# nadeemlab/DeepLIIF

Measured on AMD Instinct MI355X. Metric: 512x512 tiles/s train-step (5G+5D), higher is better.
Workload: dtype bf16; 1 GPU; DeepLIIF train step, 5x Resnet-9block G + 5x NLayerD(n=4), GAN+SmoothL1+Adam (BASELINE configs[2] per GPU); tile=512x512x3, batch_per_gpu=8, global_batch=8, norm=instance, precision_policy=bf16, parallelism=dp1, rccl_ranks=1, backend=nccl, streams=3

## Files before the change

### deepliif_amd/csrc/conv_s2d.hip

```cpp
#include "conv_args.h"

typedef __attribute__((ext_vector_type(16))) float f32x16_t;
typedef __attribute__((address_space(3))) char lds_char_t;
typedef __attribute__((address_space(3))) const bf16x8_t lds_frag_t;

__device__ __attribute__((aligned(64))) unsigned char g_s2d_zero_page[64];

template <int V> struct S2DIC { static constexpr int value = V; };

struct S2dArgs {
    ConvArgs a;
    int R, nstrips, segs;
};

constexpr int S2D_EVEN = 128 * 128;
constexpr int S2D_ODD = 136 * 128;
constexpr int S2D_SLOT = S2D_EVEN + S2D_ODD;
constexpr int S2D_TILE = 4 * S2D_SLOT;
constexpr int S2D_BIAS = S2D_TILE + 64 * 256;
constexpr size_t S2D_LDS = (size_t)S2D_BIAS + 512;
static_assert(S2D_LDS <= 160 * 1024, "LDS of one CU");

__device__ __forceinline__ float s2d_row16_sum(float v) {
    v += __builtin_bit_cast(float, __builtin_amdgcn_update_dpp(0, __builtin_bit_cast(int, v), 0xB1, 0xf, 0xf, false));
    v += __builtin_bit_cast(float, __builtin_amdgcn_update_dpp(0, __builtin_bit_cast(int, v), 0x4E, 0xf, 0xf, false));
    v += __builtin_bit_cast(float, __builtin_amdgcn_update_dpp(0, __builtin_bit_cast(int, v), 0x141, 0xf, 0xf, false));
    v += __builtin_bit_cast(float, __builtin_amdgcn_update_dpp(0, __builtin_bit_cast(int, v), 0x140, 0xf, 0xf, false));
    return v;
}

template <bool STATS, bool RELU>
__global__ void __launch_bounds__(256) conv_s2d_kernel(const S2dArgs sa) {
    const ConvArgs &a = sa.a;
    extern __shared__ __attribute__((aligned(16))) char smem_raw[];
    lds_char_t *lds = (lds_char_t *)smem_raw;

    const int tid = threadIdx.x, lane = tid & 63;
    const int wave = __builtin_amdgcn_readfirstlane(tid >> 6);
    const int lr = lane & 31, lh = lane >> 5;

    int b = blockIdx.x;
    const int strip = b % sa.nstrips; b /= sa.nstrips;
    const int seg = b % sa.segs; b /= sa.segs;
    const int tn = b % a.tiles_n;
    const int n = b / a.tiles_n;
    const int ho0 = strip * sa.R;

    bf16x8_t W[3][3][4];
    {
        const bf16_t *wp = a.w_hi + (size_t)(tn * 128 + wave * 32 + lr) * a.w_kstride + a.phase_kbase[0] + lh * 8;
#pragma unroll
        for (int kh = 0; kh < 3; ++kh)
#pragma unroll
            for (int kw = 0; kw < 3; ++kw)
#pragma unroll
                for (int s = 0; s < 4; ++s) W[kh][kw][s] = *reinterpret_cast<const bf16x8_t *>(wp + (kh * 3 + kw) * 64 + s * 16);
    }

    const int lrow = lane >> 3, lcp = lane & 7;
    const char *in = reinterpret_cast<const char *>(a.in);
    const int psb = a.in_pstride * 2;
    const unsigned OOB = 0x80000000u;
    const int pp0 = 8 * wave + lrow;
    const unsigned swz = (unsigned)((lcp ^ ((pp0 >> 1) & 7)) * 16);
    const unsigned o_off = (unsigned)((seg * 256 + 2 * pp0) * psb) + swz;
    const unsigned e_off = o_off + (unsigned)psb;
    const unsigned o_off0 = (seg * 256 + 2 * pp0 - 1 >= 0) ? o_off : OOB;
    const unsigned o_off4 = (lrow == 0) ? o_off : OOB;
    const size_t row_bytes = (size_t)a.Wi * psb;
    const __amdgpu_buffer_rsrc_t rsrc_in = __builtin_amdgcn_make_buffer_rsrc(const_cast<char *>(in + (size_t)n * a.Hi * row_bytes - psb), 0, 0x7fffffff, 0x00020000);

    const __amdgpu_buffer_rsrc_t rsrc_none = __builtin_amdgcn_make_buffer_rsrc(const_cast<char *>(in), 0, 0, 0x00020000);
    auto stage_piece = [&](auto Kc, int soff, int slot, const __amdgpu_buffer_rsrc_t rsrc_in) __attribute__((always_inline)) {
        constexpr int K = decltype(Kc)::value;
        const int dst = slot * S2D_SLOT;
        if constexpr (K < 4) {
            __builtin_amdgcn_raw_ptr_buffer_load_lds(rsrc_in, (__attribute__((address_space(3))) void *)(lds + dst + (wave + 4 * K) * 1024), 16, (int)e_off,
                                                     soff + K * 64 * psb, 0, 0);
        } else if constexpr (K < 8) {
            __builtin_amdgcn_raw_ptr_buffer_load_lds(rsrc_in, (__attribute__((address_space(3))) void *)(lds + dst + S2D_EVEN + (wave + 4 * (K - 4)) * 1024), 16,
                                                     (int)(K == 4 ? o_off0 : o_off), soff + (K - 4) * 64 * psb, 0, 0);
        } else {
            if (wave == 0)
                __builtin_amdgcn_raw_ptr_buffer_load_lds(rsrc_in, (__attribute__((address_space(3))) void *)(lds + dst + S2D_EVEN + 16 * 1024), 16, (int)o_off4,
                                                         soff + 4 * 64 * psb, 0, 0);
        }
    };
    auto stage = [&](int r, int slot) __attribute__((always_inline)) {
        const int rowp = r * (int)row_bytes;
        stage_piece(S2DIC<0>{}, rowp, slot, rsrc_in); stage_piece(S2DIC<1>{}, rowp, slot, rsrc_in); stage_piece(S2DIC<2>{}, rowp, slot, rsrc_in);
        stage_piece(S2DIC<3>{}, rowp, slot, rsrc_in); stage_piece(S2DIC<4>{}, rowp, slot, rsrc_in); stage_piece(S2DIC<5>{}, rowp, slot, rsrc_in);
        stage_piece(S2DIC<6>{}, rowp, slot, rsrc_in); stage_piece(S2DIC<7>{}, rowp, slot, rsrc_in); stage_piece(S2DIC<8>{}, rowp, slot, rsrc_in);
    };

    const int a_kw1 = lr * 128 + ((lh ^ ((lr >> 1) & 7)) << 4);
    const int a_kw0 = S2D_EVEN + a_kw1;
    const int a_kw2 = S2D_EVEN + (lr + 1) * 128 + ((lh ^ (((lr + 1) >> 1) & 7)) << 4);

    f32x16_t accA[4], accB[4];

    auto frag_base = [&](int g_kw) __attribute__((always_inline)) { return g_kw == 0 ? a_kw0 : (g_kw == 1 ? a_kw1 : a_kw2); };
    auto read_group = [&](bf16x8_t (&F)[4], int addr) __attribute__((always_inline)) {
#pragma unroll
        for (int j = 0; j < 4; ++j) F[j] = *reinterpret_cast<lds_frag_t *>(lds + addr + j * 4096);
    };
    auto row_mac = [&](auto KHC, auto KHN, int slot, int slot_next, f32x16_t (&cur)[4], f32x16_t (&nxt)[4], bf16x8_t (&F0)[4], bf16x8_t (&F1)[4],
                       int soff_dma, int slot_dma, const __amdgpu_buffer_rsrc_t rsrc_dma) __attribute__((always_inline)) {
        constexpr int khc = decltype(KHC)::value, khn = decltype(KHN)::value;
        const int base = slot * S2D_SLOT;
        auto group = [&](auto Gc, bf16x8_t (&Fc)[4], bf16x8_t (&Fn)[4]) __attribute__((always_inline)) {
            constexpr int g = decltype(Gc)::value, kw = g >> 2, sx = g & 3;
            if constexpr (g + 1 < 12) read_group(Fn, base + (frag_base((g + 1) >> 2) ^ (((g + 1) & 3) << 5)));
            else if (slot_next >= 0) read_group(Fn, slot_next * S2D_SLOT + a_kw0);
            if constexpr (g < 9) stage_piece(S2DIC<(g < 9 ? g : 0)>{}, soff_dma, slot_dma, rsrc_dma);
#pragma unroll
            for (int j = 0; j < 4; ++j) {
                if constexpr (khc >= 0) cur[j] = dl_mfma32(W[khc < 0 ? 0 : khc][kw][sx], Fc[j], cur[j]);
                if constexpr (khn >= 0) nxt[j] = dl_mfma32(W[khn < 0 ? 0 : khn][kw][sx], Fc[j], nxt[j]);
            }
        };
        group(S2DIC<0>{}, F0, F1); group(S2DIC<1>{}, F1, F0); group(S2DIC<2>{}, F0, F1); group(S2DIC<3>{}, F1, F0);
        group(S2DIC<4>{}, F0, F1); group(S2DIC<5>{}, F1, F0); group(S2DIC<6>{}, F0, F1); group(S2DIC<7>{}, F1, F0);
        group(S2DIC<8>{}, F0, F1); group(S2DIC<9>{}, F1, F0); group(S2DIC<10>{}, F0, F1); group(S2DIC<11>{}, F1, F0);
    };

    float s1[8], s2[8];
#pragma unroll
    for (int e = 0; e < 8; ++e) { s1[e] = 0.f; s2[e] = 0.f; }
    lds_char_t *tile = lds + S2D_TILE;
    const int opb = a.out_pstride * 2;
    const __amdgpu_buffer_rsrc_t rsrc_out = __builtin_amdgcn_make_buffer_rsrc(reinterpret_cast<char *>(a.out) + (size_t)n * a.Ho * a.Wo * opb, 0, 0x7fffffff, 0x00020000);
    const unsigned st_off = (unsigned)((tid >> 4) * opb + (tn * 128 + (tid & 15) * 8) * 2);
    constexpr bool relu = RELU;
    __attribute__((address_space(3))) float *bias_l = reinterpret_cast<__attribute__((address_space(3))) float *>(lds + S2D_BIAS);
    if (tid < 128) {
        const int co = tn * 128 + tid;
        bias_l[tid] = (a.bias && co < a.bias_n) ? a.bias[co] : 0.f;
    }
    __syncthreads();
    auto reset_acc = [&](f32x16_t (&acc)[4]) __attribute__((always_inline)) {
        f32x4_t bv[4];
#pragma unroll
        for (int q = 0; q < 4; ++q) bv[q] = *reinterpret_cast<__attribute__((address_space(3))) const f32x4_t *>(bias_l + wave * 32 + q * 8 + lh * 4);
#pragma unroll
        for (int j = 0; j < 4; ++j)
#pragma unroll
            for (int r = 0; r < 16; ++r) acc[j][r] = bv[r >> 2][r & 3];
    };
    reset_acc(accA);
    reset_acc(accB);

    auto epilogue = [&](f32x16_t (&acc)[4], int ho) __attribute__((always_inline)) {
        const int orow = (ho * a.Wo + seg * 128) * opb;
#pragma unroll
        for (int h = 0; h < 2; ++h) {
#pragma unroll
            for (int jj = 0; jj < 2; ++jj) {
                const int j = 2 * h + jj;
#pragma unroll
                for (int q = 0; q < 4; ++q) {
                    float v[4];
#pragma unroll
                    for (int e = 0; e < 4; ++e) {
                        v[e] = acc[j][q * 4 + e];
                        if constexpr (relu) v[e] = v[e] > 0.f ? v[e] : 0.f;
                    }
                    u32x2_t pk;
                    pk[0] = pack2_bf16(v[0], v[1]);
                    pk[1] = pack2_bf16(v[2], v[3]);
                    const int unit = (wave * 8 + q * 2 + lh) ^ ((lr & 15) << 1);
                    *reinterpret_cast<__attribute__((address_space(3))) u32x2_t *>(tile + (jj * 32 + lr) * 256 + unit * 8) = pk;
                }
            }
            asm volatile("s_waitcnt lgkmcnt(0)\n\ts_barrier" ::: "memory");
#pragma unroll
            for (int it = 0; it < 4; ++it) {
                const int idx = tid + it * 256;
                const int row = idx >> 4, cc = idx & 15;
                const int unit = (cc * 2) ^ ((row & 15) << 1);
                const u32x4_t v = *reinterpret_cast<__attribute__((address_space(3))) const u32x4_t *>(tile + row * 256 + unit * 8);
                __builtin_amdgcn_raw_buffer_store_b128(v, rsrc_out, (int)st_off, orow + (h * 64 + it * 16) * opb, 0);
                if constexpr (STATS) {
#pragma unroll
                    for (int e = 0; e < 4; ++e) {
                        const float lo = h16_lo_f32(v[e]), hi = h16_hi_f32(v[e]);
                        s1[2 * e] += lo; s2[2 * e] += lo * lo; s1[2 * e + 1] += hi; s2[2 * e + 1] += hi * hi;
                    }
                }
            }
            asm volatile("s_waitcnt lgkmcnt(0)\n\ts_barrier" ::: "memory");
        }
        reset_acc(acc);
    };

    const int R = sa.R;
    const int r_first = 2 * ho0 - 1;
    bf16x8_t FA[4], FB[4];
    if (r_first >= 0) stage(r_first, 3);
    stage(2 * ho0, 0);
    stage(2 * ho0 + 1, 1);
    asm volatile("s_waitcnt vmcnt(0)\n\ts_barrier" ::: "memory");
    if (r_first >= 0) {
        read_group(FA, 3 * S2D_SLOT + a_kw0);
        row_mac(S2DIC<0>{}, S2DIC<-1>{}, 3, -1, accA, accB, FA, FB, 0, 2, rsrc_none);
        asm volatile("s_waitcnt lgkmcnt(0)\n\ts_barrier" ::: "memory");
    }
    auto out_row = [&](int t, int s0, f32x16_t (&cur)[4], f32x16_t (&nxt)[4]) __attribute__((always_inline)) {
        const int ho = ho0 + t;
        const bool more = t + 1 < R;
        const int soff = (2 * ho + 2) * (int)row_bytes;
        read_group(FA, s0 * S2D_SLOT + a_kw0);
        const __amdgpu_buffer_rsrc_t rs = more ? rsrc_in : rsrc_none;
        row_mac(S2DIC<1>{}, S2DIC<-1>{}, s0, s0 + 1, cur, nxt, FA, FB, soff, s0 ^ 2, rs);
        row_mac(S2DIC<2>{}, S2DIC<0>{}, s0 + 1, -1, cur, nxt, FA, FB, soff + (int)row_bytes, (s0 ^ 2) + 1, rs);
        __builtin_amdgcn_sched_barrier(0);
        epilogue(cur, ho);
        __builtin_amdgcn_sched_barrier(0);
        asm volatile("s_waitcnt vmcnt(8) lgkmcnt(0)\n\ts_barrier" ::: "memory");
    };
    for (int t = 0; t < R; t += 2) {
        out_row(t, 0, accA, accB);
        out_row(t + 1, 2, accB, accA);
    }

    if constexpr (STATS) {
        __attribute__((address_space(3))) float *red = reinterpret_cast<__attribute__((address_space(3))) float *>(tile);
#pragma unroll
        for (int e = 0; e < 8; ++e) {
            float t1 = s1[e], t2 = s2[e];
            t1 += __shfl_xor(t1, 16, 64); t2 += __shfl_xor(t2, 16, 64);
            t1 += __shfl_xor(t1, 32, 64); t2 += __shfl_xor(t2, 32, 64);
            if (lane < 16) { red[(wave * 2 + 0) * 128 + lane * 8 + e] = t1; red[(wave * 2 + 1) * 128 + lane * 8 + e] = t2; }
        }
        __syncthreads();
        if (tid < 128 && tn * 128 + tid < a.Co) {
            float t1 = 0.f, t2 = 0.f;
#pragma unroll
            for (int w = 0; w < 4; ++w) { t1 += red[(w * 2 + 0) * 128 + tid]; t2 += red[(w * 2 + 1) * 128 + tid]; }
            float *o = a.stats_part + ((size_t)(n * a.stats_nchunks + seg * sa.nstrips + strip) * 2) * a.Co + tn * 128 + tid;
            o[0] = t1;
            o[a.Co] = t2;
        }
    }
}

static int s2d_strip_rows(const ConvArgs &a) {
    const int segs = a.Wo / 128, tiles_n = a.Co / 128;
    const int per_img = a.N * segs * tiles_n;
    int best = 0;
    for (int R = 2; R <= a.Ho; R += 2) {
        if (a.Ho % R) continue;
        const int wgs = per_img * (a.Ho / R);
        if (best == 0 || wgs >= 240) best = R;
        if (wgs < 240) break;
    }
    return best;
}

bool s2d_eligible(const ConvArgs &a) {
    if (a.n_phase != 1 || a.splitk != 1 || a.raw_out || a.in_step != 2 || a.out_step != 1) return false;
    if (a.phase_tap_begin[1] - a.phase_tap_begin[0] != 9 || a.Ci != 64 || a.Co < 128 || (a.Co & 127)) return false;
    if (a.Hi != 2 * a.Ho || a.Wi != 2 * a.Wo || a.Hq != a.Ho || a.Wq != a.Wo || (a.Wo & 127) || (a.Ho & 1)) return false;
    if (a.pad_mode != DL_PAD_ZERO || a.bn_y != nullptr || a.in_act != DL_ACT_NONE || a.epi_old) return false;
    if (a.act != DL_ACT_NONE && a.act != DL_ACT_RELU) return false;
    for (int t = 0; t < 9; ++t) {
        const int dh = (int)(int8_t)(a.taps[t] & 0xff), dw = (int)(int8_t)((a.taps[t] >> 8) & 0xff);
        if (dh != t / 3 - 1 || dw != t % 3 - 1) return false;
    }
    return s2d_strip_rows(a) > 0;
}

int s2d_stats_chunks(const ConvArgs &a) {
    const int R = s2d_strip_rows(a);
    return R > 0 ? (a.Wo / 128) * (a.Ho / R) : 0;
}

int launch_conv_s2d(const ConvArgs &a0, hipStream_t stream) {
    S2dArgs sa;
    memset(&sa, 0, sizeof(sa));
    sa.a = a0;
    ConvArgs &a = sa.a;
    sa.R = s2d_strip_rows(a);
    if (sa.R <= 0) DL_FAIL("dl_conv_forward(s2d): no strip height for Ho=%d", a.Ho);
    sa.nstrips = a.Ho / sa.R;
    sa.segs = a.Wo / 128;
    a.tiles_n = a.Co / 128;
    a.tiles_m = a.N * sa.segs * sa.nstrips;
    if (a.stats_part && a.stats_nchunks != sa.segs * sa.nstrips) DL_FAIL("dl_conv_forward(s2d): statistics chunks %d != %d", a.stats_nchunks, sa.segs * sa.nstrips);
    static bool attr_set = false;
    if (!attr_set) {
        hipError_t e = hipSuccess;
        const void *fns[4] = {reinterpret_cast<const void *>(conv_s2d_kernel<false, false>), reinterpret_cast<const void *>(conv_s2d_kernel<false, true>),
                              reinterpret_cast<const void *>(conv_s2d_kernel<true, false>), reinterpret_cast<const void *>(conv_s2d_kernel<true, true>)};
        for (int i = 0; i < 4 && e == hipSuccess; ++i) e = hipFuncSetAttribute(fns[i], hipFuncAttributeMaxDynamicSharedMemorySize, (int)S2D_LDS);
        if (e != hipSuccess) DL_FAIL("dl_conv_forward(s2d): hipFuncSetAttribute(%zu): %s", S2D_LDS, hipGetErrorString(e));
        attr_set = true;
    }
    dim3 grid(a.tiles_m * a.tiles_n, 1);
    const bool relu = a.act == DL_ACT_RELU;
    if (a.stats_part) {
        if (relu) hipLaunchKernelGGL((conv_s2d_kernel<true, true>), grid, dim3(256), S2D_LDS, stream, sa);
        else hipLaunchKernelGGL((conv_s2d_kernel<true, false>), grid, dim3(256), S2D_LDS, stream, sa);
    } else {
        if (relu) hipLaunchKernelGGL((conv_s2d_kernel<false, true>), grid, dim3(256), S2D_LDS, stream, sa);
        else hipLaunchKernelGGL((conv_s2d_kernel<false, false>), grid, dim3(256), S2D_LDS, stream, sa);
    }
    DL_CHECK_LAUNCH("dl_conv_forward(s2d)");
    return 0;
}
```

### deepliif_amd/csrc/conv_s2f.hip

```cpp
#include "conv_args.h"

typedef __attribute__((ext_vector_type(16))) float f32x16_t;
typedef __attribute__((address_space(3))) char lds_char_t;
typedef __attribute__((address_space(3))) const bf16x8_t lds_frag_t;

__device__ __attribute__((aligned(64))) unsigned char g_s2f_zero_page[64];

template <int V> struct S2IC { static constexpr int value = V; };

constexpr int S2F_MAX_OFF = 9;
struct S2fArgs {
    ConvArgs a;
    int n_off;
    int off_delta[S2F_MAX_OFF];
    int8_t off_dh[S2F_MAX_OFF], off_dw[S2F_MAX_OFF];
    int user_k[S2F_MAX_OFF][4];
};

__device__ __forceinline__ float s2f_row16_sum(float v) {
    v += __builtin_bit_cast(float, __builtin_amdgcn_update_dpp(0, __builtin_bit_cast(int, v), 0xB1, 0xf, 0xf, false));
    v += __builtin_bit_cast(float, __builtin_amdgcn_update_dpp(0, __builtin_bit_cast(int, v), 0x4E, 0xf, 0xf, false));
    v += __builtin_bit_cast(float, __builtin_amdgcn_update_dpp(0, __builtin_bit_cast(int, v), 0x141, 0xf, 0xf, false));
    v += __builtin_bit_cast(float, __builtin_amdgcn_update_dpp(0, __builtin_bit_cast(int, v), 0x140, 0xf, 0xf, false));
    return v;
}

constexpr int S2F_XB = 256 * 128;
constexpr int S2F_WB = 64 * 128;
constexpr int S2F_BUF = S2F_XB + 4 * S2F_WB;
constexpr size_t S2F_LOOP_LDS = (size_t)2 * S2F_BUF;
constexpr size_t S2F_EPI_LDS = (size_t)256 * 512 + 256 * sizeof(int) + (size_t)4 * 2 * 64 * sizeof(float);
constexpr size_t S2F_LDS = S2F_LOOP_LDS > S2F_EPI_LDS ? S2F_LOOP_LDS : S2F_EPI_LDS;

__global__ void __launch_bounds__(512) conv_s2f_kernel(const S2fArgs sa) {
    const ConvArgs &a = sa.a;
    extern __shared__ __attribute__((aligned(16))) char smem_raw[];
    lds_char_t *lds = (lds_char_t *)smem_raw;

    const int tid = threadIdx.x, lane = tid & 63;
    const int wave = __builtin_amdgcn_readfirstlane(tid >> 6);
    const int wm = wave & 3, wn = wave >> 2;
    const int bid = xcd_remap(blockIdx.x, gridDim.x);
    const int tn = bid % a.tiles_n, tm = bid / a.tiles_n;
    const int nch = a.Ci >> 6;
    const int NO = sa.n_off;
    const int T = nch * NO;

    const int lrow = lane >> 3, lcp = lane & 7;
    const int HWq = a.Hq * a.Wq;
    const bf16_t *in = reinterpret_cast<const bf16_t *>(a.in);
    const bf16_t *zero = reinterpret_cast<const bf16_t *>(g_s2f_zero_page);
    const bf16_t *x_ptr[4];
    unsigned x_mask[4];
#pragma unroll
    for (int i = 0; i < 4; ++i) {
        const int s = (wave * 4 + i) * 8 + lrow;
        const int m = tm * 256 + s;
        const bool ok = m < a.Mtot;
        const int mm = ok ? m : 0;
        const int n = mm / HWq, rem = mm - n * HWq;
        const int hq = rem / a.Wq, wq = rem - hq * a.Wq;
        x_ptr[i] = in + ((size_t)(n * a.Hi + hq) * a.Wi + wq) * (size_t)a.in_pstride + (lcp ^ ((s >> 1) & 7)) * 8;
        unsigned mk = 0;
        if (ok)
            for (int o = 0; o < NO; ++o) {
                const int hi = hq + sa.off_dh[o], wi = wq + sa.off_dw[o];
                if (((unsigned)hi < (unsigned)a.Hi) && ((unsigned)wi < (unsigned)a.Wi)) mk |= 1u << o;
            }
        x_mask[i] = mk;
    }
    const int wrow = wave * 8 + lrow;
    const bf16_t *w_ptr = a.w_hi + (size_t)(tn * 64 + wrow) * a.w_kstride + (lcp ^ ((wrow >> 1) & 7)) * 8;

    auto stage = [&](int u) __attribute__((always_inline)) {
        const int c = u / NO, o = u - c * NO;
        const int buf = (u & 1) * S2F_BUF;
        const ptrdiff_t xd = (ptrdiff_t)sa.off_delta[o] + c * 64;
#pragma unroll
        for (int i = 0; i < 4; ++i) {
            const bool ok = (x_mask[i] >> o) & 1u;
            const bf16_t *src = ok ? x_ptr[i] + xd : zero;
            __builtin_amdgcn_global_load_lds((const __attribute__((address_space(1))) void *)src,
                                             (__attribute__((address_space(3))) void *)(lds + buf + (wave * 4 + i) * 1024), 16, 0, 0);
        }
#pragma unroll
        for (int p = 0; p < 4; ++p) {
            const int kb = sa.user_k[o][p];
            if (kb >= 0)
                __builtin_amdgcn_global_load_lds((const __attribute__((address_space(1))) void *)(w_ptr + kb + c * 64),
                                                 (__attribute__((address_space(3))) void *)(lds + buf + S2F_XB + p * S2F_WB + wave * 1024), 16, 0, 0);
        }
    };

    const int lr = lane & 31, lh = lane >> 5;
    const int ax = (wm * 64 + lr) * 128 + ((lh ^ ((lr >> 1) & 7)) << 4);
    const int aw = S2F_XB + (wn * 32 + lr) * 128 + ((lh ^ ((lr >> 1) & 7)) << 4);

    f32x16_t acc[4][2];
#pragma unroll
    for (int p = 0; p < 4; ++p)
#pragma unroll
        for (int j = 0; j < 2; ++j)
#pragma unroll
            for (int r = 0; r < 16; ++r) acc[p][j][r] = 0.f;

    if (T > 0) stage(0);
    for (int u = 0; u < T; ++u) {
        asm volatile("s_waitcnt vmcnt(0)\n\ts_barrier" ::: "memory");
        if (u + 1 < T) stage(u + 1);
        const int c = u / NO, o = u - c * NO;
        (void)c;
        const int buf = (u & 1) * S2F_BUF;
        bf16x8_t xf[4][2];
#pragma unroll
        for (int s = 0; s < 4; ++s)
#pragma unroll
            for (int j = 0; j < 2; ++j) xf[s][j] = *reinterpret_cast<lds_frag_t *>(lds + buf + (ax ^ (s << 5)) + j * 4096);
#pragma unroll
        for (int p = 0; p < 4; ++p) {
            if (sa.user_k[o][p] < 0) continue;
            bf16x8_t wf[4];
#pragma unroll
            for (int s = 0; s < 4; ++s) wf[s] = *reinterpret_cast<lds_frag_t *>(lds + buf + p * S2F_WB + (aw ^ (s << 5)));
#pragma unroll
            for (int s = 0; s < 4; ++s)
#pragma unroll
                for (int j = 0; j < 2; ++j) acc[p][j] = dl_mfma32(wf[s], xf[s][j], acc[p][j]);
        }
    }
    asm volatile("s_waitcnt vmcnt(0) lgkmcnt(0)" ::: "memory");
    __syncthreads();

    lds_char_t *tile = lds;
    __attribute__((address_space(3))) int *rowtab = reinterpret_cast<__attribute__((address_space(3))) int *>(lds + 256 * 512);
    __attribute__((address_space(3))) float *red = reinterpret_cast<__attribute__((address_space(3))) float *>(lds + 256 * 512 + 256 * 4);
    const bool want_stats = a.stats_part != nullptr;
    if (tid < 256) {
        const int m = tm * 256 + tid;
        int opix = -1;
        if (m < a.Mtot) {
            const int n = m / HWq, rem = m - n * HWq;
            const int hq = rem / a.Wq, wq = rem - hq * a.Wq;
            opix = (n * a.Ho + 2 * hq) * a.Wo + 2 * wq;
        }
        rowtab[tid] = opix;
    }
    bool live[2];
#pragma unroll
    for (int j = 0; j < 2; ++j) live[j] = tm * 256 + wm * 64 + j * 32 + lr < a.Mtot;
#pragma unroll
    for (int q = 0; q < 4; ++q) {
        const int cl = wn * 32 + q * 8 + lh * 4;
        const int co = tn * 64 + cl;
        float bias[4] = {0.f, 0.f, 0.f, 0.f};
        if (a.bias) {
#pragma unroll
            for (int e = 0; e < 4; ++e) bias[e] = (co + e < a.bias_n) ? a.bias[co + e] : 0.f;
        }
        float s1[4] = {0.f, 0.f, 0.f, 0.f}, s2[4] = {0.f, 0.f, 0.f, 0.f};
#pragma unroll
        for (int p = 0; p < 4; ++p) {
            const int vch = p * 64 + cl;
            const int unit = (vch >> 2) ^ (((lr & 15) << 1) & 62);
#pragma unroll
            for (int j = 0; j < 2; ++j) {
                float v[4];
#pragma unroll
                for (int e = 0; e < 4; ++e) v[e] = acc[p][j][q * 4 + e] + bias[e];
                if (a.act == DL_ACT_RELU) {
#pragma unroll
                    for (int e = 0; e < 4; ++e) v[e] = v[e] > 0.f ? v[e] : 0.f;
                }
                u32x2_t pk;
                pk[0] = pack2_bf16(v[0], v[1]);
                pk[1] = pack2_bf16(v[2], v[3]);
                *reinterpret_cast<__attribute__((address_space(3))) u32x2_t *>(tile + (wm * 64 + j * 32 + lr) * 512 + unit * 8) = pk;
                if (want_stats && live[j]) {
                    const float q0 = h16_lo_f32(pk[0]), q1 = h16_hi_f32(pk[0]);
                    const float q2 = h16_lo_f32(pk[1]), q3 = h16_hi_f32(pk[1]);
                    s1[0] += q0; s2[0] += q0 * q0; s1[1] += q1; s2[1] += q1 * q1;
                    s1[2] += q2; s2[2] += q2 * q2; s1[3] += q3; s2[3] += q3 * q3;
                }
            }
        }
        if (want_stats) {
#pragma unroll
            for (int e = 0; e < 4; ++e) {
                s1[e] = s2f_row16_sum(s1[e]); s2[e] = s2f_row16_sum(s2[e]);
                s1[e] += __shfl_xor(s1[e], 16, 64); s2[e] += __shfl_xor(s2[e], 16, 64);
            }
            if (lr == 0) {
#pragma unroll
                for (int e = 0; e < 4; ++e) {
                    red[(wm * 2 + 0) * 64 + cl + e] = s1[e];
                    red[(wm * 2 + 1) * 64 + cl + e] = s2[e];
                }
            }
        }
    }
    __syncthreads();
    bf16_t *out = reinterpret_cast<bf16_t *>(a.out);
#pragma unroll 4
    for (int idx = tid; idx < 256 * 32; idx += 512) {
        const int row = idx >> 5, cc = idx & 31;
        const int opix = rowtab[row];
        const int p = cc >> 3, co = tn * 64 + (cc & 7) * 8;
        if (opix < 0 || co >= a.Co) continue;
        const int unit = (cc * 2) ^ (((row & 15) << 1) & 62);
        const u32x4_t v = *reinterpret_cast<__attribute__((address_space(3))) const u32x4_t *>(tile + row * 512 + unit * 8);
        *reinterpret_cast<u32x4_t *>(out + ((size_t)opix + (size_t)(p >> 1) * a.Wo + (p & 1)) * a.out_pstride + co) = v;
    }
    if (want_stats && tid < 64) {
        const int m0 = tm * 256;
        const int n = m0 / HWq;
        const int chunk = (m0 - n * HWq) >> 8;
        const int co = tn * 64 + tid;
        if (co < a.Co) {
            float t1 = 0.f, t2 = 0.f;
#pragma unroll
            for (int w = 0; w < 4; ++w) { t1 += red[(w * 2 + 0) * 64 + tid]; t2 += red[(w * 2 + 1) * 64 + tid]; }
            float *o = a.stats_part + ((size_t)(n * a.stats_nchunks + chunk) * 2) * a.Co + co;
            o[0] = t1;
            o[a.Co] = t2;
        }
    }
}

static bool s2f_phase_order_ok(const ConvArgs &a) {
    for (int p = 0; p < 4; ++p)
        if (a.phase_oh[p] != (p >> 1) || a.phase_ow[p] != (p & 1)) return false;
    return true;
}

bool s2f_eligible(const ConvArgs &a) {
    if (a.n_phase != 4 || a.splitk != 1 || a.raw_out || a.in_step != 1 || a.out_step != 2 || !s2f_phase_order_ok(a)) return false;
    if (a.Ho != 2 * a.Hq || a.Wo != 2 * a.Wq || a.Hi != a.Hq || a.Wi != a.Wq) return false;
    if (a.Ci < 64 || (a.Ci & 63) || a.Co < 64 || (a.Co & 63) || a.pad_mode != DL_PAD_ZERO || a.bn_y != nullptr || a.in_act != DL_ACT_NONE) return false;
    if (a.act != DL_ACT_NONE && a.act != DL_ACT_RELU) return false;
    if (a.epi_old) return false;
    const char *env = dl_switch(DL_SW_CONV_S2F);
    if (a.Mtot < 65536 && !(env && env[0] == '2')) return false;
    int ndist = 0;
    int16_t seen[S2F_MAX_OFF + 1];
    for (int t = 0; t < a.phase_tap_begin[4]; ++t) {
        bool dup = false;
        for (int i = 0; i < ndist; ++i) dup |= seen[i] == a.taps[t];
        if (!dup) {
            if (ndist == S2F_MAX_OFF) return false;
            seen[ndist++] = a.taps[t];
        }
    }
    for (int p = 0; p < 4; ++p)
        for (int t = a.phase_tap_begin[p]; t < a.phase_tap_begin[p + 1]; ++t)
            for (int t2 = t + 1; t2 < a.phase_tap_begin[p + 1]; ++t2)
                if (a.taps[t] == a.taps[t2]) return false;
    return ndist > 0;
}

int s2f_stats_chunks(const ConvArgs &a) {
    const int hw = a.Hq * a.Wq;
    return (hw % 256) ? 0 : hw / 256;
}

int launch_conv_s2f(const ConvArgs &a0, hipStream_t stream) {
    S2fArgs sa;
    memset(&sa, 0, sizeof(sa));
    sa.a = a0;
    ConvArgs &a = sa.a;
    a.tiles_m = (a.Mtot + 255) / 256;
    a.tiles_n = a.Co / 64;
    int no = 0;
    int16_t key[S2F_MAX_OFF];
    for (int p = 0; p < 4; ++p)
        for (int t = a.phase_tap_begin[p]; t < a.phase_tap_begin[p + 1]; ++t) {
            int o = -1;
            for (int i = 0; i < no; ++i)
                if (key[i] == a.taps[t]) o = i;
            if (o < 0) {
                o = no++;
                key[o] = a.taps[t];
                sa.off_dh[o] = (int8_t)(a.taps[t] & 0xff);
                sa.off_dw[o] = (int8_t)((a.taps[t] >> 8) & 0xff);
                sa.off_delta[o] = ((int)sa.off_dh[o] * a.Wi + (int)sa.off_dw[o]) * a.in_pstride;
                for (int q = 0; q < 4; ++q) sa.user_k[o][q] = -1;
            }
            sa.user_k[o][p] = a.phase_kbase[p] + (t - a.phase_tap_begin[p]) * a.Ci;
        }
    sa.n_off = no;
    static bool attr_set = false;
    if (!attr_set) {
        hipError_t e = hipFuncSetAttribute(reinterpret_cast<const void *>(conv_s2f_kernel), hipFuncAttributeMaxDynamicSharedMemorySize, (int)S2F_LDS);
        if (e != hipSuccess) DL_FAIL("dl_conv_forward(s2f): hipFuncSetAttribute(%zu): %s", S2F_LDS, hipGetErrorString(e));
        attr_set = true;
    }
    dim3 grid(a.tiles_m * a.tiles_n, 1);
    hipLaunchKernelGGL(conv_s2f_kernel, grid, dim3(512), S2F_LDS, stream, sa);
    DL_CHECK_LAUNCH("dl_conv_forward(s2f)");
    return 0;
}
```

Measured before the change: 117.5 tiles/s.

## Share input slabs across horizontal tap offsets in s2f transposed conv

Groups the tap offsets of the stride-2 transposed-conv kernel by their row shift. For each row group it stages one 264-row input slab, with halo rows for the neighbouring pixels, and reads the -1/0/+1 column shifts from that slab by re-indexing LDS rows. Weight tiles move to an 8-slot ring buffer so one offset's weights no longer force a full slab reload. The aim is to cut redundant global-to-LDS input traffic, up to three loads per group of offsets. In exchange the host planning is more complex, eligibility gains a pipelining-distance check and a 2GB size check, and correctness depends on careful handling of the halo and row-boundary masks.

```diff
diff --git a/deepliif_amd/csrc/conv_s2d.hip b/deepliif_amd/csrc/conv_s2d.hip
--- a/deepliif_amd/csrc/conv_s2d.hip
+++ b/deepliif_amd/csrc/conv_s2d.hip
@@ -263,6 +263,7 @@
     if (a.Hi != 2 * a.Ho || a.Wi != 2 * a.Wo || a.Hq != a.Ho || a.Wq != a.Wo || (a.Wo & 127) || (a.Ho & 1)) return false;
     if (a.pad_mode != DL_PAD_ZERO || a.bn_y != nullptr || a.in_act != DL_ACT_NONE || a.epi_old) return false;
     if (a.act != DL_ACT_NONE && a.act != DL_ACT_RELU) return false;
+    if ((size_t)a.Hi * a.Wi * (size_t)a.in_pstride * 2 >= ((size_t)1 << 31) || (size_t)a.Ho * a.Wo * (size_t)a.out_pstride * 2 >= ((size_t)1 << 31)) return false;
     for (int t = 0; t < 9; ++t) {
         const int dh = (int)(int8_t)(a.taps[t] & 0xff), dw = (int)(int8_t)((a.taps[t] >> 8) & 0xff);
         if (dh != t / 3 - 1 || dw != t % 3 - 1) return false;
diff --git a/deepliif_amd/csrc/conv_s2f.hip b/deepliif_amd/csrc/conv_s2f.hip
--- a/deepliif_amd/csrc/conv_s2f.hip
+++ b/deepliif_amd/csrc/conv_s2f.hip
@@ -11,11 +11,14 @@
 constexpr int S2F_MAX_OFF = 9;
 struct S2fArgs {
     ConvArgs a;
-    int n_off;
-    int off_delta[S2F_MAX_OFF];
-    int8_t off_dh[S2F_MAX_OFF], off_dw[S2F_MAX_OFF];
+    int n_off, n_grp;
+    int tpc;
+    int grp_delta[S2F_MAX_OFF];
+    int grp_dh[S2F_MAX_OFF];
+    unsigned off_info[S2F_MAX_OFF];
     int user_k[S2F_MAX_OFF][4];
 };
+__host__ __device__ constexpr unsigned s2f_info(unsigned i, int lo, int bits) { return (i >> lo) & ((1u << bits) - 1u); }
 
 __device__ __forceinline__ float s2f_row16_sum(float v) {
     v += __builtin_bit_cast(float, __builtin_amdgcn_update_dpp(0, __builtin_bit_cast(int, v), 0xB1, 0xf, 0xf, false));
@@ -25,12 +28,17 @@
     return v;
 }
 
-constexpr int S2F_XB = 256 * 128;
+constexpr int S2F_SROWS = 264;
+constexpr int S2F_XB = S2F_SROWS * 128;
 constexpr int S2F_WB = 64 * 128;
-constexpr int S2F_BUF = S2F_XB + 4 * S2F_WB;
-constexpr size_t S2F_LOOP_LDS = (size_t)2 * S2F_BUF;
+constexpr int S2F_W0 = 2 * S2F_XB;
+constexpr int S2F_SLOTS = 8;
+constexpr size_t S2F_LOOP_LDS = (size_t)S2F_W0 + (size_t)S2F_SLOTS * S2F_WB;
 constexpr size_t S2F_EPI_LDS = (size_t)256 * 512 + 256 * sizeof(int) + (size_t)4 * 2 * 64 * sizeof(float);
 constexpr size_t S2F_LDS = S2F_LOOP_LDS > S2F_EPI_LDS ? S2F_LOOP_LDS : S2F_EPI_LDS;
+static_assert(S2F_LDS <= 160 * 1024, "the whole LDS of a CU");
+
+constexpr int S2F_VMCNT0 = 0x0F70;
 
 __global__ void __launch_bounds__(512) conv_s2f_kernel(const S2fArgs sa) {
     const ConvArgs &a = sa.a;
@@ -43,58 +51,82 @@
     const int bid = xcd_remap(blockIdx.x, gridDim.x);
     const int tn = bid % a.tiles_n, tm = bid / a.tiles_n;
     const int nch = a.Ci >> 6;
-    const int NO = sa.n_off;
+    const int NO = sa.n_off, NG = sa.n_grp;
     const int T = nch * NO;
 
     const int lrow = lane >> 3, lcp = lane & 7;
     const int HWq = a.Hq * a.Wq;
     const bf16_t *in = reinterpret_cast<const bf16_t *>(a.in);
     const bf16_t *zero = reinterpret_cast<const bf16_t *>(g_s2f_zero_page);
+    auto slab_src = [&](int m, int r, unsigned &mask) __attribute__((always_inline)) {
+        mask = 0;
+        if (m < 0 || m >= a.Mtot) return zero;
+        const int n = m / HWq, rem = m - n * HWq;
+        const int hq = rem / a.Wq, wq = rem - hq * a.Wq;
+        for (int g = 0; g < NG; ++g)
+            if ((unsigned)(hq + sa.grp_dh[g]) < (unsigned)a.Hi) mask |= 1u << g;
+        return in + ((size_t)(n * a.Hi + hq) * a.Wi + wq) * (size_t)a.in_pstride + (lcp ^ ((r >> 1) & 7)) * 8;
+    };
     const bf16_t *x_ptr[4];
     unsigned x_mask[4];
 #pragma unroll
     for (int i = 0; i < 4; ++i) {
         const int s = (wave * 4 + i) * 8 + lrow;
-        const int m = tm * 256 + s;
-        const bool ok = m < a.Mtot;
-        const int mm = ok ? m : 0;
-        const int n = mm / HWq, rem = mm - n * HWq;
-        const int hq = rem / a.Wq, wq = rem - hq * a.Wq;
-        x_ptr[i] = in + ((size_t)(n * a.Hi + hq) * a.Wi + wq) * (size_t)a.in_pstride + (lcp ^ ((s >> 1) & 7)) * 8;
-        unsigned mk = 0;
-        if (ok)
-            for (int o = 0; o < NO; ++o) {
-                const int hi = hq + sa.off_dh[o], wi = wq + sa.off_dw[o];
-                if (((unsigned)hi < (unsigned)a.Hi) && ((unsigned)wi < (unsigned)a.Wi)) mk |= 1u << o;
-            }
-        x_mask[i] = mk;
-    }
+        x_ptr[i] = slab_src(tm * 256 + s, s, x_mask[i]);
+    }
+    unsigned h_mask = 0;
+    const bf16_t *h_ptr = zero;
+    if (wave == 0 && lane < 16) h_ptr = slab_src(lane < 8 ? tm * 256 + 256 : tm * 256 - 1, lane < 8 ? 256 : 257, h_mask);
     const int wrow = wave * 8 + lrow;
     const bf16_t *w_ptr = a.w_hi + (size_t)(tn * 64 + wrow) * a.w_kstride + (lcp ^ ((wrow >> 1) & 7)) * 8;
 
     auto stage = [&](int u) __attribute__((always_inline)) {
         const int c = u / NO, o = u - c * NO;
-        const int buf = (u & 1) * S2F_BUF;
-        const ptrdiff_t xd = (ptrdiff_t)sa.off_delta[o] + c * 64;
-#pragma unroll
-        for (int i = 0; i < 4; ++i) {
-            const bool ok = (x_mask[i] >> o) & 1u;
-            const bf16_t *src = ok ? x_ptr[i] + xd : zero;
-            __builtin_amdgcn_global_load_lds((const __attribute__((address_space(1))) void *)src,
-                                             (__attribute__((address_space(3))) void *)(lds + buf + (wave * 4 + i) * 1024), 16, 0, 0);
-        }
+        const unsigned inf = sa.off_info[o];
+        if (s2f_info(inf, 10, 1)) {
+            const int g = s2f_info(inf, 6, 4);
+            const int sb = ((c * NG + g) & 1) * S2F_XB;
+            const ptrdiff_t xd = (ptrdiff_t)sa.grp_delta[g] + c * 64;
+#pragma unroll
+            for (int i = 0; i < 4; ++i) {
+                const bool ok = (x_mask[i] >> g) & 1u;
+                const bf16_t *src = ok ? x_ptr[i] + xd : zero;
+                __builtin_amdgcn_global_load_lds((const __attribute__((address_space(1))) void *)src,
+                                                 (__attribute__((address_space(3))) void *)(lds + sb + (wave * 4 + i) * 1024), 16, 0, 0);
+            }
+            if (wave == 0) {
+                const bool ok = (h_mask >> g) & 1u;
+                const bf16_t *src = ok ? h_ptr + xd : zero;
+                __builtin_amdgcn_global_load_lds((const __attribute__((address_space(1))) void *)src,
+                                                 (__attribute__((address_space(3))) void *)(lds + sb + 256 * 128), 16, 0, 0);
+            }
+        }
+        const int t0 = c * sa.tpc + s2f_info(inf, 16, 6);
 #pragma unroll
         for (int p = 0; p < 4; ++p) {
-            const int kb = sa.user_k[o][p];
-            if (kb >= 0)
-                __builtin_amdgcn_global_load_lds((const __attribute__((address_space(1))) void *)(w_ptr + kb + c * 64),
-                                                 (__attribute__((address_space(3))) void *)(lds + buf + S2F_XB + p * S2F_WB + wave * 1024), 16, 0, 0);
+            if (s2f_info(inf, p, 1))
+                __builtin_amdgcn_global_load_lds((const __attribute__((address_space(1))) void *)(w_ptr + sa.user_k[o][p] + c * 64),
+                                                 (__attribute__((address_space(3))) void *)(lds + S2F_W0 + ((t0 + s2f_info(inf, 22 + 2 * p, 2)) & (S2F_SLOTS - 1)) * S2F_WB +
+                                                                                           wave * 1024), 16, 0, 0);
         }
     };
 
     const int lr = lane & 31, lh = lane >> 5;
-    const int ax = (wm * 64 + lr) * 128 + ((lh ^ ((lr >> 1) & 7)) << 4);
-    const int aw = S2F_XB + (wn * 32 + lr) * 128 + ((lh ^ ((lr >> 1) & 7)) << 4);
+    int ax[3][2];
+#pragma unroll
+    for (int j = 0; j < 2; ++j) {
+        const int s = wm * 64 + j * 32 + lr;
+        const int m = tm * 256 + s;
+        const int wq = m < a.Mtot ? (m % HWq) % a.Wq : 1;
+#pragma unroll
+        for (int d = 0; d < 3; ++d) {
+            const int sr = s + d - 1;
+            const bool off_row = (d == 0 && wq == 0) || (d == 2 && wq == a.Wq - 1);
+            const int r = off_row ? 258 : (sr < 0 ? 257 : sr);
+            ax[d][j] = r * 128 + ((lh ^ ((r >> 1) & 7)) << 4);
+        }
+    }
+    const int aw = (wn * 32 + lr) * 128 + ((lh ^ ((lr >> 1) & 7)) << 4);
 
     f32x16_t acc[4][2];
 #pragma unroll
@@ -106,29 +138,38 @@
 
     if (T > 0) stage(0);
     for (int u = 0; u < T; ++u) {
-        asm volatile("s_waitcnt vmcnt(0)\n\ts_barrier" ::: "memory");
+        __builtin_amdgcn_sched_barrier(0);
+        __builtin_amdgcn_s_waitcnt(S2F_VMCNT0);
+        __builtin_amdgcn_s_barrier();
+        __builtin_amdgcn_sched_barrier(0);
         if (u + 1 < T) stage(u + 1);
+        __builtin_amdgcn_sched_barrier(0);
         const int c = u / NO, o = u - c * NO;
-        (void)c;
-        const int buf = (u & 1) * S2F_BUF;
+        const unsigned inf = sa.off_info[o];
+        const int sb = ((c * NG + (int)s2f_info(inf, 6, 4)) & 1) * S2F_XB;
+        const int t0 = c * sa.tpc + s2f_info(inf, 16, 6);
+        const int dsel = s2f_info(inf, 4, 2);
         bf16x8_t xf[4][2];
 #pragma unroll
-        for (int s = 0; s < 4; ++s)
-#pragma unroll
-            for (int j = 0; j < 2; ++j) xf[s][j] = *reinterpret_cast<lds_frag_t *>(lds + buf + (ax ^ (s << 5)) + j * 4096);
+        for (int j = 0; j < 2; ++j) {
+            const int axj = dsel == 0 ? ax[0][j] : (dsel == 2 ? ax[2][j] : ax[1][j]);
+#pragma unroll
+            for (int s = 0; s < 4; ++s) xf[s][j] = *reinterpret_cast<lds_frag_t *>(lds + sb + (axj ^ (s << 5)));
+        }
 #pragma unroll
         for (int p = 0; p < 4; ++p) {
-            if (sa.user_k[o][p] < 0) continue;
+            if (!s2f_info(inf, p, 1)) continue;
             bf16x8_t wf[4];
-#pragma unroll
-            for (int s = 0; s < 4; ++s) wf[s] = *reinterpret_cast<lds_frag_t *>(lds + buf + p * S2F_WB + (aw ^ (s << 5)));
+            const int wb = S2F_W0 + ((t0 + s2f_info(inf, 22 + 2 * p, 2)) & (S2F_SLOTS - 1)) * S2F_WB;
+#pragma unroll
+            for (int s = 0; s < 4; ++s) wf[s] = *reinterpret_cast<lds_frag_t *>(lds + wb + (aw ^ (s << 5)));
 #pragma unroll
             for (int s = 0; s < 4; ++s)
 #pragma unroll
                 for (int j = 0; j < 2; ++j) acc[p][j] = dl_mfma32(wf[s], xf[s][j], acc[p][j]);
         }
     }
-    asm volatile("s_waitcnt vmcnt(0) lgkmcnt(0)" ::: "memory");
+    __builtin_amdgcn_sched_barrier(0);
     __syncthreads();
 
     lds_char_t *tile = lds;
@@ -232,29 +273,74 @@
     return true;
 }
 
+static bool s2f_plan(const ConvArgs &a, S2fArgs &sa) {
+    int no = 0;
+    int16_t key[S2F_MAX_OFF];
+    int odh[S2F_MAX_OFF], odw[S2F_MAX_OFF], uk[S2F_MAX_OFF][4], ntap[S2F_MAX_OFF];
+    for (int p = 0; p < 4; ++p)
+        for (int t = a.phase_tap_begin[p]; t < a.phase_tap_begin[p + 1]; ++t) {
+            int o = -1;
+            for (int i = 0; i < no; ++i)
+                if (key[i] == a.taps[t]) o = i;
+            if (o < 0) {
+                if (no == S2F_MAX_OFF) return false;
+                o = no++;
+                key[o] = a.taps[t];
+                odh[o] = (int8_t)(a.taps[t] & 0xff);
+                odw[o] = (int8_t)((a.taps[t] >> 8) & 0xff);
+                ntap[o] = 0;
+                for (int q = 0; q < 4; ++q) uk[o][q] = -1;
+            }
+            if (uk[o][p] >= 0) return false;
+            if (odw[o] < -1 || odw[o] > 1) return false;
+            uk[o][p] = a.phase_kbase[p] + (t - a.phase_tap_begin[p]) * a.Ci;
+            ++ntap[o];
+        }
+    if (no == 0) return false;
+    int ng = 0, tpc = 0;
+    int gfirst[S2F_MAX_OFF], glast[S2F_MAX_OFF];
+    for (int o = 0; o < no; ++o) {
+        int g = 0;
+        while (g < ng && sa.grp_dh[g] != odh[o]) ++g;
+        const bool first = g == ng;
+        if (first) {
+            sa.grp_dh[ng] = odh[o];
+            sa.grp_delta[ng] = odh[o] * a.Wi * a.in_pstride;
+            gfirst[ng] = o;
+            ++ng;
+        }
+        glast[g] = o;
+        unsigned inf = ((unsigned)(odw[o] + 1) << 4) | ((unsigned)g << 6) | ((first ? 1u : 0u) << 10) | ((unsigned)tpc << 16);
+        int r = 0;
+        for (int q = 0; q < 4; ++q) {
+            sa.user_k[o][q] = uk[o][q];
+            if (uk[o][q] >= 0) inf |= (1u << q) | ((unsigned)r++ << (22 + 2 * q));
+        }
+        sa.off_info[o] = inf;
+        tpc += ntap[o];
+    }
+    for (int i = 2; i < 3 * ng; ++i) {
+        const int c = i / ng, g = i % ng, c2 = (i - 2) / ng, g2 = (i - 2) % ng;
+        if (c2 * no + glast[g2] > c * no + gfirst[g] - 2) return false;
+    }
+    sa.n_off = no;
+    sa.n_grp = ng;
+    sa.tpc = tpc;
+    return true;
+}
+
 bool s2f_eligible(const ConvArgs &a) {
     if (a.n_phase != 4 || a.splitk != 1 || a.raw_out || a.in_step != 1 || a.out_step != 2 || !s2f_phase_order_ok(a)) return false;
     if (a.Ho != 2 * a.Hq || a.Wo != 2 * a.Wq || a.Hi != a.Hq || a.Wi != a.Wq) return false;
     if (a.Ci < 64 || (a.Ci & 63) || a.Co < 64 || (a.Co & 63) || a.pad_mode != DL_PAD_ZERO || a.bn_y != nullptr || a.in_act != DL_ACT_NONE) return false;
     if (a.act != DL_ACT_NONE && a.act != DL_ACT_RELU) return false;
     if (a.epi_old) return false;
+    if ((size_t)a.N * a.Hi * a.Wi * (size_t)a.in_pstride * 2 >= ((size_t)1 << 31) || (size_t)a.N * a.Ho * a.Wo * (size_t)a.out_pstride * 2 >= ((size_t)1 << 31)) return false;
     const char *env = dl_switch(DL_SW_CONV_S2F);
     if (a.Mtot < 65536 && !(env && env[0] == '2')) return false;
-    int ndist = 0;
-    int16_t seen[S2F_MAX_OFF + 1];
-    for (int t = 0; t < a.phase_tap_begin[4]; ++t) {
-        bool dup = false;
-        for (int i = 0; i < ndist; ++i) dup |= seen[i] == a.taps[t];
-        if (!dup) {
-            if (ndist == S2F_MAX_OFF) return false;
-            seen[ndist++] = a.taps[t];
-        }
-    }
-    for (int p = 0; p < 4; ++p)
-        for (int t = a.phase_tap_begin[p]; t < a.phase_tap_begin[p + 1]; ++t)
-            for (int t2 = t + 1; t2 < a.phase_tap_begin[p + 1]; ++t2)
-                if (a.taps[t] == a.taps[t2]) return false;
-    return ndist > 0;
+    S2fArgs sa;
+    memset(&sa, 0, sizeof(sa));
+    return s2f_plan(a, sa);
 }
 
 int s2f_stats_chunks(const ConvArgs &a) {
@@ -269,24 +355,7 @@
     ConvArgs &a = sa.a;
     a.tiles_m = (a.Mtot + 255) / 256;
     a.tiles_n = a.Co / 64;
-    int no = 0;
-    int16_t key[S2F_MAX_OFF];
-    for (int p = 0; p < 4; ++p)
-        for (int t = a.phase_tap_begin[p]; t < a.phase_tap_begin[p + 1]; ++t) {
-            int o = -1;
-            for (int i = 0; i < no; ++i)
-                if (key[i] == a.taps[t]) o = i;
-            if (o < 0) {
-                o = no++;
-                key[o] = a.taps[t];
-                sa.off_dh[o] = (int8_t)(a.taps[t] & 0xff);
-                sa.off_dw[o] = (int8_t)((a.taps[t] >> 8) & 0xff);
-                sa.off_delta[o] = ((int)sa.off_dh[o] * a.Wi + (int)sa.off_dw[o]) * a.in_pstride;
-                for (int q = 0; q < 4; ++q) sa.user_k[o][q] = -1;
-            }
-            sa.user_k[o][p] = a.phase_kbase[p] + (t - a.phase_tap_begin[p]) * a.Ci;
-        }
-    sa.n_off = no;
+    if (!s2f_plan(a, sa)) DL_FAIL("dl_conv_forward(s2f): no K-step plan for these taps");
     static bool attr_set = false;
     if (!attr_set) {
         hipError_t e = hipFuncSetAttribute(reinterpret_cast<const void *>(conv_s2f_kernel), hipFuncAttributeMaxDynamicSharedMemorySize, (int)S2F_LDS);
```

Result: no change. 118.1 tiles/s (median of 6 runs) (+0.5%).
